# CSU-KangHu/HiTE

Measured on AMD Instinct MI355X. Metric: candidate TE boundaries/sec on 1 Gbp synthetic genome (fine stage: copy finding+gather+align+vote+judge), higher is better.
Workload: dtype u8; 1 GPU; C3: 1000 Mbp synthetic genome, 2500 TIR + 2500 LTR families, 50000 candidates/GPU judged as TIR (copy finding by minimizer-index lookup inside the timed step; index build 0.0 s untimed); genome_bp=1000000000, candidates_per_gpu=50000, candidate_bases=192511237, copies=799813, copy_table=found, is_te=34225, parallelism=replicated genome, candidates per rank x1, all-gather of 32-B calls

## Files before the change

hite_amd/_lib.py:

```python
import ctypes as C
import os

import numpy as np

_HERE = os.path.dirname(os.path.abspath(__file__))
SO_PATH = os.path.join(_HERE, "libhite_gpu.so")

HITE_TE = {"tir": 0, "helitron": 1, "non_ltr": 2}
INFO = {0: "", 1: "nb", 2: "fl1", 3: "EXC"}
HITE_SUBCLUSTER_CHUNK = 64


class HiteError(RuntimeError):
    pass


class HiteCall(C.Structure):
    _fields_ = [("is_te", C.c_int32), ("info", C.c_int32), ("row_num", C.c_int32), ("bstart", C.c_int32),
                ("bend", C.c_int32), ("cons_len", C.c_int32), ("cons_off", C.c_int64)]


CALL_DTYPE = np.dtype([("is_te", "<i4"), ("info", "<i4"), ("row_num", "<i4"), ("bstart", "<i4"), ("bend", "<i4"),
                       ("cons_len", "<i4"), ("cons_off", "<i8")])
assert CALL_DTYPE.itemsize == 32 and C.sizeof(HiteCall) == 32
# ... 151 lines not shown
        return [counts[coff[i]:coff[i + 1]] for i in range(len(msas))]

    def boundary_search(self, msas, pos, side, thr, variant=3, int_thr=None, out_thr=None, win_in=20, win_out=10):
        buf, off, rows, cols = self.pack_msas(msas)
        n = len(msas)
        pos = _arr(pos, np.int32)
        side = _arr([0 if s in (0, "start") else 1 for s in side], np.int32)
        thr = _arr(thr, np.float64)
        it = _arr(int_thr, np.float64) if int_thr is not None else None
        ot = _arr(out_thr, np.float64) if out_thr is not None else None
        b = np.zeros(n, dtype=np.int32)
        v = np.zeros(n, dtype=np.int32)
        self._check(self.lib.hite_boundary_search(self.h, n, _p(buf), _p(off), _p(rows), _p(cols), _p(pos), _p(side), _p(thr),
                                                  _p(it), _p(ot), int(variant), win_in, win_out, _p(b), _p(v)),
                    "hite_boundary_search")
        return b, v

    def judge(self, te_type, msas, cands, plant=1):
        buf, off, rows, cols = self.pack_msas(msas)
        n = len(msas)
        cb = [c.encode() if isinstance(c, str) else bytes(c) for c in cands]
        coff = np.zeros(n + 1, dtype=np.int64)
        np.cumsum([len(c) for c in cb], out=coff[1:])
        cbuf = np.frombuffer(b"".join(cb) + b"\0" * 16, dtype=np.uint8)
        calls = np.zeros(n, dtype=CALL_DTYPE)
        cons = np.zeros(int(cols.astype(np.int64).sum()) + 8 * n + 16, dtype=np.uint8)
        self._check(self.lib.hite_judge(self.h, HITE_TE[te_type], int(plant), n, _p(buf), _p(off), _p(rows), _p(cols),
                                        _p(cbuf), _p(coff), _p(calls), _p(cons)), "hite_judge")
        out = []
        for i in range(n):
            c = calls[i]
            s = cons[c["cons_off"]:c["cons_off"] + c["cons_len"]].tobytes().decode() if c["is_te"] else ""
            out.append((bool(c["is_te"]), INFO[int(c["info"])], s, int(c["row_num"]), int(c["bstart"]), int(c["bend"])))
        return out

    def tsd_search(self, rows_, bstart, bend, plant=1):
        rb = [r.encode() if isinstance(r, str) else bytes(r) for r in rows_]
        n = len(rb)
        off = np.zeros(n + 1, dtype=np.int64)
        np.cumsum([len(r) for r in rb], out=off[1:])
        buf = np.frombuffer(b"".join(rb) + b"\0" * 16, dtype=np.uint8)
        ln = np.zeros(n, dtype=np.int32)
        lo = np.zeros((n, 16), dtype=np.uint8)
        ro = np.zeros((n, 16), dtype=np.uint8)
        self._check(self.lib.hite_tsd_search(self.h, n, _p(buf), _p(off), _p(_arr(bstart, np.int32)), _p(_arr(bend, np.int32)),
                                             int(plant), _p(ln), _p(lo), _p(ro)), "hite_tsd_search")
        return [(lo[i, :max(ln[i], 0)].tobytes().decode(), ro[i, :max(ln[i], 0)].tobytes().decode(), int(ln[i])) for i in range(n)]

    def align_config(self, exact_cap):
        self._check(self.lib.hite_align_config(self.h, int(exact_cap)), "hite_align_config")

    def align_lanes(self, min_cols):
        self._check(self.lib.hite_align_lanes(self.h, int(min_cols)), "hite_align_lanes")

    def align_stats(self, reset=False):
        o = np.zeros(8, dtype=np.int64)
        self._check(self.lib.hite_align_stats(self.h, _p(o), 1 if reset else 0), "hite_align_stats")
        return dict(zip(("pairs", "certified", "wide", "fallback", "dropped", "cost", "columns", "exact_cap"), (int(x) for x in o)))

    def star_msa(self, groups, sparse=False, info=False):
        flat = [w.encode() if isinstance(w, str) else bytes(w) for g in groups for w in g]
        n = len(groups)
        row_first = np.zeros(n + 1, dtype=np.int32)
        np.cumsum([len(g) for g in groups], out=row_first[1:])
        off = np.zeros(len(flat) + 1, dtype=np.int64)
        np.cumsum([len(w) for w in flat], out=off[1:])
        buf = np.frombuffer(b"".join(flat) + b"\0" * 16, dtype=np.uint8)
        cols = np.zeros(n, dtype=np.int32)
        rows = np.zeros(n, dtype=np.int32)
        inf = np.zeros((len(flat), 5), dtype=np.int32)
        moff = np.zeros(max(n, 1), dtype=np.int64)
        if n == 0:
            return ([], []) if info else []
        ptr = C.POINTER(C.c_uint8)()
        nbytes = C.c_int64(0)
        self._check(self.lib.hite_star_msa_once(self.h, n, _p(buf), _p(off), _p(row_first), 1 if sparse else 0, _p(cols), _p(rows),
                                                _p(inf) if info else None, C.byref(ptr), _p(moff), C.byref(nbytes)), "hite_star_msa_once")
        try:
            out = np.ctypeslib.as_array(ptr, shape=(max(int(nbytes.value), 1),)).copy() if nbytes.value > 0 else np.zeros(1, dtype=np.uint8)
        finally:
            self.lib.hite_host_free(C.cast(ptr, C.c_void_p))
        res = []
        for i in range(n):
            if cols[i] <= 0:
                res.append(None)
            else:
                res.append(out[moff[i]:moff[i] + int(rows[i]) * cols[i]].reshape(int(rows[i]), int(cols[i])).copy())
        if info:
            return res, [inf[row_first[i]:row_first[i + 1]].copy() for i in range(n)]
        return res

    def flank_region_align(self, te_type, cands, copies, plant=1, flank=50):
        n = len(cands)
        cb = [c.encode() if isinstance(c, str) else bytes(c) for c in cands]
        coff = np.zeros(n + 1, dtype=np.int64)
        np.cumsum([len(c) for c in cb], out=coff[1:])
        cbuf = np.frombuffer(b"".join(cb) + b"\0" * 16, dtype=np.uint8)
        cf = np.zeros(n + 1, dtype=np.int32)
        np.cumsum([len(c) for c in copies], out=cf[1:])
        flat = [t for c in copies for t in c]
        contig = _arr([t[0] for t in flat], np.int32)
        s1 = _arr([t[1] for t in flat], np.int64)
        e1 = _arr([t[2] for t in flat], np.int64)
        mn = _arr([t[3] for t in flat], np.uint8)
        has = [len(t) > 5 for t in flat]
        if any(has) and not all(has):
# ... 619 lines not shown
```

hite_amd/csrc/hite_align.hip:

```cpp
#include "hite_common.h"
#include "hite_scan.h"
#include "hite_arena.h"
#include "hite_sort.h"
#include "hite_align.h"

#define AL_GAP 3
#define AL_STEER 24
#define AL_MARGIN 48
#define AL_PADR 1056
#define AL_WIDE_NW 64
#define AL_STRIP 16
#define AL_RECB 4096
#define AL_DEFAULT_CAP 8
#define AL_KBINS 2048
#define AL_LANES_MIN_STRIPS 32

struct AlignArgs {
    const uint8_t *win;
    const int64_t *win_off;
    const int32_t *win_len;
    const int32_t *row_first;
    int n_cand;
    const int32_t *row_cand;
    const uint4 *planes;
// ... 1247 lines not shown
        __syncthreads();
    }
    if (fail) { if (lane == 0) P.st[g] = 1; }
    else out.run(i - 1, i, 0x8000u);
}

__global__ void align_flag_kernel(int64_t nrows, const int32_t *__restrict__ order, const int32_t *__restrict__ strips, AlignArgs P,
                                  int what, int level, int cap, int32_t *__restrict__ flag, int32_t *__restrict__ cols) {
    const int64_t x = (int64_t)blockIdx.x * blockDim.x + threadIdx.x;
    if (x >= nrows) return;
    const int g = order[x];
    int f = 0;
    if (strips[g] > 0) {
        if (what == 0) {
            const int u4 = P.U4[g];
            if (P.st[g] == 0 && u4 >= 0 && u4 + AL_GAP * AL_MARGIN <= 32 * AL_GAP * cap) {
                int first = 8;
                while (32 * AL_GAP * first < u4 + AL_GAP * AL_MARGIN) first *= 2;
                const bool cert = P.U[g] <= P.kst[g];
                f = level >= first && !cert;
            }
        } else if (what == 1) f = P.st[g] == 1;
        else {
            const int u4 = P.U4[g];
            const bool esc = P.st[g] == 0 && u4 >= 0 && u4 + AL_GAP * AL_MARGIN <= 32 * AL_GAP * cap && !(P.U[g] <= P.kst[g]);
            f = what == 2 ? esc : !esc;
        }
    }
    flag[x] = f;
    if (cols) cols[x] = f ? P.win_len[g] + 1 : 0;
}
__global__ void align_compact_kernel(int64_t nrows, const int32_t *__restrict__ order, const int32_t *__restrict__ flag,
                                     const int64_t *__restrict__ pos, int32_t *__restrict__ out, const int64_t *__restrict__ colpos,
                                     int64_t *__restrict__ full_off, int32_t *__restrict__ st) {
    const int64_t x = (int64_t)blockIdx.x * blockDim.x + threadIdx.x;
    if (x >= nrows) return;
    if (flag[x]) {
        const int g = order[x];
        out[pos[x]] = g;
        if (full_off) { full_off[g] = colpos[x]; st[g] = 0; }
    }
}
__global__ void __launch_bounds__(256) align_blockmax_kernel(int64_t cnt, const int32_t *__restrict__ list, const int32_t *__restrict__ strips,
                                                             int32_t *__restrict__ bk) {
    const int64_t x = (int64_t)blockIdx.x * 256 + threadIdx.x;
    const int k = wave_max_i32(x < cnt ? strips[list[x]] : 0);
    if ((threadIdx.x & 63) == 0 && x < cnt) bk[x >> 6] = k;
}
__global__ void align_assign_kernel(int64_t cnt, const int32_t *__restrict__ list, const int64_t *__restrict__ boff, char *region,
                                    unsigned long long *__restrict__ rec) {
    const int64_t x = (int64_t)blockIdx.x * blockDim.x + threadIdx.x;
    if (x < cnt) rec[list[x]] = (unsigned long long)(uintptr_t)(region + boff[x >> 6] * (int64_t)AL_RECB + (x & 63) * 32);
}
struct LaneCost { float thread_chain, lane_chain, thread_work, lane_work; };
__device__ __forceinline__ double lane_cost_at(int64_t k, int64_t nb, const int32_t *bk, const int64_t *boff, const LaneCost c) {
    const double chain_l = k > 0 ? (double)bk[0] * c.lane_chain : 0.0, chain_t = k < nb ? (double)bk[k] * c.thread_chain : 0.0;
    const double work = (double)boff[k] * c.lane_work + (double)(boff[nb] - boff[k]) * c.thread_work;
    double t = chain_l > chain_t ? chain_l : chain_t;
    return t > work ? t : work;
}
__global__ void align_long_blocks_kernel(int64_t nb, const int32_t *__restrict__ bk, const int64_t *__restrict__ boff, int64_t fixed_strips,
                                         LaneCost cf, LaneCost ct, int64_t *__restrict__ out) {
    if (blockIdx.x || threadIdx.x) return;
    for (int w = 0; w < 2; w++) {
        int64_t lo = 0, hi = nb;
        if (fixed_strips >= 0) {
            while (lo < hi) { const int64_t mid = (lo + hi) >> 1; if ((int64_t)bk[mid] >= fixed_strips) lo = mid + 1; else hi = mid; }
        } else {
            const LaneCost c = w ? ct : cf;
            while (lo < hi) {
                const int64_t mid = (lo + hi) >> 1;
                const double a = (double)bk[0] * c.lane_chain, wk = (double)boff[mid] * c.lane_work + (double)(boff[nb] - boff[mid]) * c.thread_work;
                const double tc = mid < nb ? (double)bk[mid] * c.thread_chain : 0.0;
                if ((a > wk ? a : wk) < tc) lo = mid + 1; else hi = mid;
            }
            if (lo > 0 && lane_cost_at(lo - 1, nb, bk, boff, c) <= lane_cost_at(lo, nb, bk, boff, c)) lo--;
            if (lo > 0 && (bk[0] < AL_LANES_MIN_STRIPS || lane_cost_at(lo, nb, bk, boff, c) > 0.9 * lane_cost_at(0, nb, bk, boff, c))) lo = 0;
        }
        out[w] = lo;
    }
}
__global__ void __launch_bounds__(256) align_stats_kernel(int64_t total_rows, const int32_t *__restrict__ strips, AlignArgs P, int32_t *__restrict__ row_dead,
                                                          int32_t *__restrict__ cand_status, unsigned long long *__restrict__ acc) {
    __shared__ unsigned long long s_acc[4][7];
    unsigned long long v[7] = {0, 0, 0, 0, 0, 0, 0};
    for (int64_t g = (int64_t)blockIdx.x * blockDim.x + threadIdx.x; g < total_rows; g += (int64_t)gridDim.x * blockDim.x) {
        if (strips[g] <= 0) {
            const bool empty_row = g != P.row_first[P.row_cand[g]];
            if (empty_row) { P.st[g] = 2; P.U[g] = -1; P.kst[g] = -1; P.lvl[g] = 0; v[0] += 1ull; v[4] += 1ull; }
            if (row_dead) row_dead[g] = empty_row;
            if (empty_row && cand_status) atomicExch(&cand_status[P.row_cand[g]], 2);
        }
        else {
            const int st = P.st[g];
            v[0] += 1ull;
            v[1] += st == 0 && P.U[g] <= P.kst[g];
            v[2] += st == 0 && (P.lvl[g] & 0xff) > 4;
            v[3] += (P.lvl[g] & 0x100) != 0;
            v[4] += st != 0;
            v[5] += st == 0 ? (unsigned long long)P.U[g] : 0ull;
            v[6] += (unsigned long long)P.win_len[g];
            if (row_dead) row_dead[g] = st != 0;
            if (st != 0 && cand_status) atomicExch(&cand_status[P.row_cand[g]], 2);
        }
    }
#pragma unroll
    for (int q = 0; q < 7; q++) {
        unsigned long long x = v[q];
#pragma unroll
        for (int d = 32; d >= 1; d >>= 1) x += __shfl_xor(x, d, 64);
        if ((threadIdx.x & 63) == 0) s_acc[threadIdx.x >> 6][q] = x;
    }
    __syncthreads();
    if (threadIdx.x < 7) {
        const unsigned long long x = s_acc[0][threadIdx.x] + s_acc[1][threadIdx.x] + s_acc[2][threadIdx.x] + s_acc[3][threadIdx.x];
        if (x) atomicAdd(&acc[threadIdx.x], x);
    }
}
__global__ void align_info_kernel(int64_t total_rows, AlignArgs P, int32_t *__restrict__ info ) {
    const int64_t g = (int64_t)blockIdx.x * blockDim.x + threadIdx.x;
    if (g >= total_rows) return;
    const int c = P.row_cand[g];
    if (g == P.row_first[c]) { for (int q = 0; q < 5; q++) info[g * 5 + q] = 0; return; }
    info[g * 5 + 0] = P.U[g];
    info[g * 5 + 1] = P.st[g] != 2 && P.U[g] <= P.kst[g];
    info[g * 5 + 2] = P.st[g];
    info[g * 5 + 3] = P.kst[g];
    info[g * 5 + 4] = P.lvl[g];
}

struct AlignState {
    Arena arena;
    int64_t *h_pin = nullptr;
    int64_t *d_scal = nullptr;
    int exact_cap = -1;
    int lanes_min = -1;
    float lanes_scale[4] = {1.f, 1.f, 1.f, 1.f};
    bool sort_attr = false;
    hipStream_t st2 = nullptr;
    hipEvent_t ev = nullptr, ev_fork = nullptr, ev_join = nullptr;
    int64_t stats[8] = {0, 0, 0, 0, 0, 0, 0, 0};
};

static hipError_t align_make_stream(hipStream_t *out) {
    int lo = 0, hi = 0;
    if (hipDeviceGetStreamPriorityRange(&lo, &hi) != hipSuccess) { lo = 0; hi = 0; }
    return hipStreamCreateWithPriority(out, hipStreamNonBlocking, hi);
}

static AlignState *align_state(hite_ctx *ctx) {
    if (!ctx->align_state) {
        AlignState *S = new AlignState();
        if (hipHostMalloc((void **)&S->h_pin, 64 * sizeof(int64_t)) != hipSuccess || hipMalloc((void **)&S->d_scal, 64 * sizeof(int64_t)) != hipSuccess ||
            align_make_stream(&S->st2) != hipSuccess || hipEventCreateWithFlags(&S->ev, hipEventDisableTiming) != hipSuccess ||
            hipEventCreateWithFlags(&S->ev_fork, hipEventDisableTiming) != hipSuccess || hipEventCreateWithFlags(&S->ev_join, hipEventDisableTiming) != hipSuccess) {
            delete S;
            return nullptr;
        }
        const char *e = getenv("HITE_ALIGN_EXACT");
        int cap = e && *e ? atoi(e) : AL_DEFAULT_CAP;
        if (cap != 0 && cap != 8 && cap != 16 && cap != 32) cap = AL_DEFAULT_CAP;
        S->exact_cap = cap;
        const char *l = getenv("HITE_ALIGN_LANES");
        if (l && *l) { const int v = atoi(l); S->lanes_min = v < -2 ? -1 : v; }
        const char *sc = getenv("HITE_ALIGN_LANES_SCALE");
        if (sc && *sc) sscanf(sc, "%f,%f,%f,%f", &S->lanes_scale[0], &S->lanes_scale[1], &S->lanes_scale[2], &S->lanes_scale[3]);
        ctx->align_state = S;
    }
    return (AlignState *)ctx->align_state;
}
void hite_align_release(hite_ctx *ctx) {
    AlignState *S = (AlignState *)ctx->align_state;
    if (!S) return;
    arena_free(S->arena);
    if (S->h_pin) (void)hipHostFree(S->h_pin);
    if (S->d_scal) (void)hipFree(S->d_scal);
    if (S->st2) (void)hipStreamDestroy(S->st2);
    if (S->ev) (void)hipEventDestroy(S->ev);
    if (S->ev_fork) (void)hipEventDestroy(S->ev_fork);
    if (S->ev_join) (void)hipEventDestroy(S->ev_join);
    delete S;
    ctx->align_state = nullptr;
}

extern "C" int hite_align_config(hite_ctx *ctx, int32_t exact_cap) {
    if (!ctx || (exact_cap != 0 && exact_cap != 8 && exact_cap != 16 && exact_cap != 32)) return HITE_EINVAL;
    AlignState *S = align_state(ctx);
    if (!S) return HITE_ENOMEM;
    S->exact_cap = exact_cap;
    return HITE_OK;
}
extern "C" int hite_align_lanes(hite_ctx *ctx, int32_t min_cols) {
    if (!ctx || min_cols < -2 || min_cols > 32767) return HITE_EINVAL;
    AlignState *S = align_state(ctx);
    if (!S) return HITE_ENOMEM;
    S->lanes_min = min_cols;
    return HITE_OK;
}
extern "C" int hite_align_stats(hite_ctx *ctx, int64_t *out8, int32_t reset) {
    if (!ctx || !out8) return HITE_EINVAL;
    AlignState *S = align_state(ctx);
    if (!S) return HITE_ENOMEM;
    memcpy(out8, S->stats, sizeof S->stats);
    out8[7] = S->exact_cap;
    if (reset) memset(S->stats, 0, sizeof S->stats);
    return HITE_OK;
}

#define ACHK(x) do { int rc__ = (x); if (rc__) return rc__; } while (0)

template <typename T>
static int aalloc(hite_ctx *ctx, Arena &A, size_t count, T **out) {
    void *p = nullptr;
    int rc = arena_alloc(ctx, A, count * sizeof(T), &p);
    *out = (T *)p;
    return rc;
}

static int build_list(hite_ctx *ctx, AlignState *S, hipStream_t st, int64_t nrows, const int32_t *order, const int32_t *strips,
                      AlignArgs &P, int what, int level, int cap, int32_t *flag, int32_t *cols, int64_t *pos, int64_t *colpos,
                      int64_t *scan_tmp, int32_t *list, int64_t *full_off, int64_t *count, int64_t *total_cols, int slot = 0) {
    const unsigned nb = (unsigned)((nrows + 255) / 256);
    hipLaunchKernelGGL(align_flag_kernel, dim3(nb), dim3(256), 0, st, nrows, order, strips, P, what, level, cap, flag, cols);
    ACHK(scan_excl_buf<int32_t>(ctx, scan_tmp, flag, nrows, pos, st));
    if (cols) ACHK(scan_excl_buf<int32_t>(ctx, scan_tmp, cols, nrows, colpos, st));
    hipLaunchKernelGGL(align_compact_kernel, dim3(nb), dim3(256), 0, st, nrows, order, flag, pos, list, cols ? colpos : nullptr,
                       cols ? full_off : nullptr, P.st);
    HITE_CHECK(ctx, hipMemcpyAsync(S->d_scal + slot, pos + nrows, 8, hipMemcpyDeviceToDevice, st));
    if (cols) HITE_CHECK(ctx, hipMemcpyAsync(S->d_scal + slot + 1, colpos + nrows, 8, hipMemcpyDeviceToDevice, st));
    HITE_CHECK(ctx, hipMemcpyAsync(S->h_pin + slot, S->d_scal + slot, 16, hipMemcpyDeviceToHost, st));
    HITE_CHECK(ctx, hipStreamSynchronize(st));
    *count = S->h_pin[slot];
    if (total_cols) *total_cols = cols ? S->h_pin[slot + 1] : 0;
    return HITE_OK;
}

static int assign_records(hite_ctx *ctx, AlignState *S, hipStream_t st, const int32_t *list, int64_t cnt, const int32_t *strips, int32_t *bk,
                          int64_t *boff, int64_t *scan_tmp, unsigned long long *rec, int slot, int words = 4, int64_t *n_long = nullptr, int64_t *n_long_tb = nullptr) {
    if (n_long) *n_long = 0;
    if (n_long_tb) *n_long_tb = 0;
    if (cnt <= 0) return HITE_OK;
    const int64_t nb = (cnt + 63) / 64;
    hipLaunchKernelGGL(align_blockmax_kernel, dim3((unsigned)((cnt + 255) / 256)), dim3(256), 0, st, cnt, list, strips, bk);
    ACHK(scan_excl_buf<int32_t>(ctx, scan_tmp, bk, nb, boff, st));
    HITE_CHECK(ctx, hipMemcpyAsync(S->d_scal + slot, boff + nb, 8, hipMemcpyDeviceToDevice, st));
    const bool lanes = n_long && S->lanes_min != -2;
    if (lanes) {
        LaneCost fwd4 = {5440.f, 3200.f, 4.3f, 12.5f}, fwd8 = {7040.f, 3200.f, 13.75f, 25.f}, tb = {6880.f, 530.f, 4.3f, 21.5f};
        fwd4.lane_work *= S->lanes_scale[0]; fwd8.lane_work *= S->lanes_scale[1]; tb.lane_work *= S->lanes_scale[2];
        fwd4.lane_chain *= S->lanes_scale[3]; fwd8.lane_chain *= S->lanes_scale[3];
        hipLaunchKernelGGL(align_long_blocks_kernel, dim3(1), dim3(1), 0, st, nb, bk, boff,
                           (int64_t)(S->lanes_min < 0 ? -1 : (S->lanes_min + AL_STRIP - 1) / AL_STRIP), words == 4 ? fwd4 : fwd8, tb, S->d_scal + slot + 1);
    }
    HITE_CHECK(ctx, hipMemcpyAsync(S->h_pin + slot, S->d_scal + slot, 24, hipMemcpyDeviceToHost, st));
    HITE_CHECK(ctx, hipStreamSynchronize(st));
    const int64_t block_strips = S->h_pin[slot];
    if (lanes) {
        const int64_t v = S->h_pin[slot + 1] * 64, vt = S->h_pin[slot + 2] * 64;
        *n_long = v < cnt ? v : cnt;
        if (n_long_tb) *n_long_tb = vt < cnt ? vt : cnt;
    }
    char *region;
    ACHK(aalloc(ctx, S->arena, (size_t)block_strips * AL_RECB + 256, &region));
    hipLaunchKernelGGL(align_assign_kernel, dim3((unsigned)((cnt + 255) / 256)), dim3(256), 0, st, cnt, list, boff, region, rec);
    return HITE_OK;
}

int hite_align_run(hite_ctx *ctx, int32_t n_cand, const uint8_t *d_win, const int64_t *d_win_off, const int32_t *d_win_len,
                   const int32_t *d_row_first, int64_t total_rows, const int64_t *d_ops_base, uint16_t *d_ops,
                   int32_t *d_row_dead, int32_t *d_cand_flag, int32_t *d_info, const char *tag, hipStream_t st) {
    if (!ctx || n_cand < 0 || total_rows < 0 || total_rows > 0x7fffffff) return HITE_EINVAL;
    if (n_cand == 0 || total_rows == 0) return HITE_OK;
    AlignState *S = align_state(ctx);
    if (!S) return HITE_ENOMEM;
    Arena &A = S->arena;
    ACHK(arena_reset(ctx, A, true));
    const int cap = S->exact_cap;
    AlignArgs P;
    memset(&P, 0, sizeof P);
    P.win = d_win; P.win_off = d_win_off; P.win_len = d_win_len; P.row_first = d_row_first; P.n_cand = n_cand;
    P.ops_base = d_ops_base; P.ops = d_ops;
    int32_t *row_cand, *strips, *order, *pwords, *flag, *flag2, *cols, *list, *list_esc, *list_fin;
    unsigned long long *skeys;
    int64_t *plane_off, *pos, *pos2, *colpos, *scan_tmp, *scan_tmp2, *full_off, *boff, *boff2;
    int32_t *bk, *bk2;
    unsigned long long *rec;
    ACHK(aalloc(ctx, A, (size_t)total_rows, &row_cand));
    ACHK(aalloc(ctx, A, (size_t)total_rows, &strips));
    ACHK(aalloc(ctx, A, (size_t)total_rows + 1, &skeys));
    ACHK(aalloc(ctx, A, (size_t)total_rows + 1, &order));
    Sorter srt;
    srt.ctx = ctx; srt.st = st; srt.cap = total_rows; srt.hist_n = sorter_hist_elems(total_rows);
    ACHK(aalloc(ctx, A, (size_t)total_rows + 1, &srt.k2));
    ACHK(aalloc(ctx, A, (size_t)total_rows + 1, &srt.v2));
    ACHK(aalloc(ctx, A, (size_t)srt.hist_n, &srt.hist));
    ACHK(aalloc(ctx, A, (size_t)srt.hist_n + 1, &srt.offs));
    ACHK(aalloc(ctx, A, (size_t)sorter_tmp_elems(srt.hist_n), &srt.bs));
    ACHK(aalloc(ctx, A, (size_t)n_cand, &pwords));
    ACHK(aalloc(ctx, A, (size_t)n_cand + 1, &plane_off));
    ACHK(aalloc(ctx, A, (size_t)total_rows, &rec));
    ACHK(aalloc(ctx, A, (size_t)total_rows / 64 + 2, &bk));
    ACHK(aalloc(ctx, A, (size_t)total_rows / 64 + 3, &boff));
    ACHK(aalloc(ctx, A, (size_t)total_rows / 64 + 2, &bk2));
    ACHK(aalloc(ctx, A, (size_t)total_rows / 64 + 3, &boff2));
    ACHK(aalloc(ctx, A, (size_t)total_rows, &flag));
    ACHK(aalloc(ctx, A, (size_t)total_rows, &cols));
    ACHK(aalloc(ctx, A, (size_t)total_rows, &list));
    ACHK(aalloc(ctx, A, (size_t)total_rows, &list_esc));
    ACHK(aalloc(ctx, A, (size_t)total_rows, &list_fin));
    ACHK(aalloc(ctx, A, (size_t)total_rows, &flag2));
    ACHK(aalloc(ctx, A, (size_t)total_rows + 1, &pos2));
    ACHK(aalloc(ctx, A, (size_t)scan_tmp_elems(total_rows) + 16, &scan_tmp2));
    ACHK(aalloc(ctx, A, (size_t)total_rows + 1, &pos));
// ... 10 lines not shown
    HITE_CHECK(ctx, hipMemsetAsync(P.st, 0, (size_t)total_rows * 4, st));
    HITE_CHECK(ctx, hipMemsetAsync(P.lvl, 0, (size_t)total_rows * 4, st));
    hipLaunchKernelGGL(align_rows_kernel, dim3(n_cand), dim3(256), 0, st, n_cand, d_row_first, d_win_len, row_cand, strips, skeys, (unsigned *)order);
    if (!S->sort_attr) {
        HITE_CHECK(ctx, hipFuncSetAttribute(reinterpret_cast<const void *>(rs_scatter_staged_kernel<true>), hipFuncAttributeMaxDynamicSharedMemorySize, RSS_LDS_BYTES));
        S->sort_attr = true;
    }
    ACHK(sorter_sort(srt, skeys, (unsigned *)order, total_rows, 11));
    hipLaunchKernelGGL(align_plane_words_kernel, dim3((n_cand + 255) / 256), dim3(256), 0, st, n_cand, d_row_first, d_win_len, pwords);
    ACHK(scan_excl_buf<int32_t>(ctx, scan_tmp, pwords, n_cand, plane_off, st));
    HITE_CHECK(ctx, hipMemcpyAsync(S->d_scal, plane_off + n_cand, 8, hipMemcpyDeviceToDevice, st));
    HITE_CHECK(ctx, hipMemcpyAsync(S->h_pin, S->d_scal, 8, hipMemcpyDeviceToHost, st));
    int64_t nl4 = 0, nltb = 0;
    ACHK(assign_records(ctx, S, st, order, total_rows, strips, bk, boff, scan_tmp, rec, 1, 4, &nl4, &nltb));
    const int64_t plane_words = S->h_pin[0];
    uint4 *planes;
    ACHK(aalloc(ctx, A, (size_t)plane_words + 8, &planes));
    P.planes = planes; P.plane_off = plane_off; P.rec = rec;
    hipLaunchKernelGGL(align_planes_kernel, dim3(n_cand), dim3(256), 0, st, n_cand, d_win, d_win_off, d_win_len, d_row_first, plane_off, planes);
    hite_prof_end(ctx, tk, st);
    HITE_CHECK(ctx, hipGetLastError());
    char name[32];
    const int nrows = (int)total_rows;
    snprintf(name, sizeof name, "align_fwd4%s", tag ? tag : "");
    hipStream_t s2 = S->st2;
    char lname[40];
    if (getenv("HITE_ALIGN_DEBUG")) fprintf(stderr, "[align%s] rows %d  block-strips %lld  lane-parallel prefix %lld forward, %lld traceback\n", tag ? tag : "", nrows, (long long)S->h_pin[1], (long long)nl4, (long long)nltb);
    if (nl4 > 0) {
        HITE_CHECK(ctx, hipEventRecord(S->ev_fork, st));
        HITE_CHECK(ctx, hipStreamWaitEvent(s2, S->ev_fork, 0));
        snprintf(lname, sizeof lname, "align_fwd4_lanes%s", tag ? tag : "");
        const int tl = hite_prof_begin(ctx, lname, s2);
        hipLaunchKernelGGL(HIP_KERNEL_NAME(align_fwd_lanes_kernel<4>), dim3((unsigned)((nl4 + 15) / 16)), dim3(64), 0, s2, P, order, (int)nl4);
        hite_prof_end(ctx, tl, s2);
        HITE_CHECK(ctx, hipEventRecord(S->ev_join, s2));
    }
    if (nrows > nl4) {
        tk = hite_prof_begin(ctx, name, st);
        hipLaunchKernelGGL(align_fwd4_kernel, dim3((unsigned)((nrows - nl4 + 63) / 64)), dim3(64), 0, st, P, order + nl4, (int)(nrows - nl4));
        hite_prof_end(ctx, tk, st);
    }
    if (nl4 > 0) HITE_CHECK(ctx, hipStreamWaitEvent(st, S->ev_join, 0));
    snprintf(name, sizeof name, "align_tb%s", tag ? tag : "");
    char wname[32];
    snprintf(wname, sizeof wname, "align_fwd_wide%s", tag ? tag : "");
    int64_t n_esc = 0, n_fin = 0;
    const bool overlap = cap >= 16;
    if (cap >= 8 && !overlap) {
        tk = hite_prof_begin(ctx, wname, st);
        for (int level = 8; level <= cap; level *= 2) {
            int64_t cnt = 0;
            ACHK(build_list(ctx, S, st, total_rows, order, strips, P, 0, level, cap, flag, nullptr, pos, colpos, scan_tmp, list, nullptr, &cnt, nullptr));
            if (cnt == 0) continue;
            int64_t nl8 = 0;
            ACHK(assign_records(ctx, S, st, list, cnt, strips, bk, boff, scan_tmp, rec, 1, 8, &nl8));
            if (getenv("HITE_ALIGN_DEBUG")) fprintf(stderr, "[align%s] level %d: pairs %lld  block-strips %lld  lane-parallel prefix %lld\n", tag ? tag : "", level, (long long)cnt, (long long)S->h_pin[1], (long long)nl8);
            if (nl8 > 0) {
                HITE_CHECK(ctx, hipEventRecord(S->ev_fork, st));
                HITE_CHECK(ctx, hipStreamWaitEvent(s2, S->ev_fork, 0));
                snprintf(lname, sizeof lname, "align_fwd_wide_lanes%s", tag ? tag : "");
                const int tl = hite_prof_begin(ctx, lname, s2);
                hipLaunchKernelGGL(HIP_KERNEL_NAME(align_fwd_lanes_kernel<8>), dim3((unsigned)((nl8 + 7) / 8)), dim3(64), 0, s2, P, list, (int)nl8);
                hite_prof_end(ctx, tl, s2);
                HITE_CHECK(ctx, hipEventRecord(S->ev_join, s2));
            }
            if (cnt > nl8)
                hipLaunchKernelGGL(align_fwd8_pair_kernel, dim3((unsigned)((cnt - nl8 + 31) / 32)), dim3(64), 0, st, P, list + nl8, (int)(cnt - nl8));
            if (nl8 > 0) HITE_CHECK(ctx, hipStreamWaitEvent(st, S->ev_join, 0));
        }
        hite_prof_end(ctx, tk, st);
    }
    if (overlap) {
        ACHK(build_list(ctx, S, st, total_rows, order, strips, P, 2, 0, cap, flag, nullptr, pos, colpos, scan_tmp, list_esc, nullptr, &n_esc, nullptr));
        if (n_esc > 0)
            ACHK(build_list(ctx, S, st, total_rows, order, strips, P, 3, 0, cap, flag, nullptr, pos, colpos, scan_tmp, list_fin, nullptr, &n_fin, nullptr));
    }
    if (n_esc > 0) {
        if (n_fin > 0) {
            tk = hite_prof_begin(ctx, name, st);
            hipLaunchKernelGGL(align_tb_kernel, dim3((unsigned)((n_fin + 63) / 64)), dim3(64), 0, st, P, list_fin, (int)n_fin);
            hite_prof_end(ctx, tk, st);
        }
        tk = hite_prof_begin(ctx, wname, s2);
        for (int level = 8; level <= cap; level *= 2) {
            int64_t cnt = 0;
            ACHK(build_list(ctx, S, s2, total_rows, order, strips, P, 0, level, cap, flag2, nullptr, pos2, colpos, scan_tmp2, list, nullptr, &cnt, nullptr, 8));
            if (cnt == 0) continue;
            ACHK(assign_records(ctx, S, s2, list, cnt, strips, bk2, boff2, scan_tmp2, rec, 10));
            const dim3 grid((unsigned)((cnt + 63) / 64));
            if (level == 8) hipLaunchKernelGGL(HIP_KERNEL_NAME(align_fwd_kernel<8>), grid, dim3(64), 0, s2, P, list, (int)cnt);
            else if (level == 16) hipLaunchKernelGGL(HIP_KERNEL_NAME(align_fwd_kernel<16>), grid, dim3(64), 0, s2, P, list, (int)cnt);
            else hipLaunchKernelGGL(HIP_KERNEL_NAME(align_fwd_kernel<32>), grid, dim3(64), 0, s2, P, list, (int)cnt);
        }
        hite_prof_end(ctx, tk, s2);
        HITE_CHECK(ctx, hipEventRecord(S->ev, s2));
        HITE_CHECK(ctx, hipStreamWaitEvent(st, S->ev, 0));
        tk = hite_prof_begin(ctx, name, st);
        hipLaunchKernelGGL(align_tb_kernel, dim3((unsigned)((n_esc + 63) / 64)), dim3(64), 0, st, P, list_esc, (int)n_esc);
        hite_prof_end(ctx, tk, st);
    } else {
        if (nltb > 0) {
            HITE_CHECK(ctx, hipEventRecord(S->ev_fork, st));
            HITE_CHECK(ctx, hipStreamWaitEvent(s2, S->ev_fork, 0));
            snprintf(lname, sizeof lname, "align_tb_strips%s", tag ? tag : "");
            const int tl = hite_prof_begin(ctx, lname, s2);
            hipLaunchKernelGGL(align_tb_strips_kernel, dim3((unsigned)nltb), dim3(64), 0, s2, P, order, (int)nltb);
            hite_prof_end(ctx, tl, s2);
            HITE_CHECK(ctx, hipEventRecord(S->ev_join, s2));
        }
        if (nrows > nltb) {
            tk = hite_prof_begin(ctx, name, st);
            hipLaunchKernelGGL(align_tb_kernel, dim3((unsigned)((nrows - nltb + 63) / 64)), dim3(64), 0, st, P, order + nltb, (int)(nrows - nltb));
            hite_prof_end(ctx, tk, st);
        }
        if (nltb > 0) HITE_CHECK(ctx, hipStreamWaitEvent(st, S->ev_join, 0));
    }
    HITE_CHECK(ctx, hipGetLastError());
    {
        int64_t cnt = 0, tcols = 0;
        ACHK(build_list(ctx, S, st, total_rows, order, strips, P, 1, 0, cap, flag, cols, pos, colpos, scan_tmp, list, full_off, &cnt, &tcols));
        if (cnt > 0) {
// ... 19 lines not shown
```

include/hite_gpu.h:

```cpp
#ifndef HITE_GPU_H
#define HITE_GPU_H
#include <stdint.h>

#ifdef __cplusplus
extern "C" {
#endif

#define HITE_ROW_PAD 0x2e
#define HITE_IS_ROW_PAD(c) (((c) & 0x20u) != 0)

#define HITE_OK 0
#define HITE_EINVAL (-1)
#define HITE_ENOMEM (-2)
#define HITE_EHIP (-3)
#define HITE_ECAP (-4)
#define HITE_ENODEV (-5)

#define HITE_TE_TIR 0
#define HITE_TE_HELITRON 1
#define HITE_TE_NON_LTR 2

#define HITE_INFO_NONE 0
#define HITE_INFO_NB 1
#define HITE_INFO_FL1 2
// ... 116 lines not shown
                        double min_identity, int32_t min_len, int32_t match, int32_t mismatch, int32_t gap_open, int32_t gap_extend,
                        int32_t *d_out, void *stream);

int hite_translate6(hite_ctx *ctx, int64_t n, const uint8_t *nt, const int64_t *nt_off, int64_t cap, uint8_t *aa_out, int64_t *frame_off);
int hite_protein_lib_build(hite_ctx *ctx, int64_t n_prot, const uint8_t *aa, const int64_t *aa_off, void **state_io);
void hite_protein_lib_release(void *state);
int hite_protein_search(hite_ctx *ctx, void *state, int64_t n_query, const uint8_t *nt, const int64_t *nt_off, double evalue, int64_t cap,
                        int32_t *o_query, int32_t *o_prot, int32_t *o_frame, int32_t *o_qstart, int32_t *o_qend, int32_t *o_sstart,
                        int32_t *o_send, int32_t *o_score, int32_t *o_ident, int32_t *o_cols, int64_t *n_out, int64_t *stats);
int hite_protein_smin(int64_t m, int64_t n, double evalue, int32_t *smin);
int hite_protein_tasks(int64_t n, const int32_t *frame, const int32_t *prot, const int32_t *diag, const int32_t *seg_start,
                       const int32_t *seg_end, int64_t n_frames, const int32_t *frame_len, int64_t cap, int32_t *o_frame, int32_t *o_prot,
                       int32_t *o_c, int32_t *o_lo, int32_t *o_hi, int64_t *n_out);
int hite_protein_hsp_filter(int64_t n, const int32_t *score, const int32_t *f_start, const int32_t *p_start, const int32_t *f_end,
                            const int32_t *p_end, uint8_t *keep);

#define HITE_IDENT_MAX_WIDTH 2048
int hite_pair_identity(hite_ctx *ctx, int64_t n_seq, const uint8_t *seqs, const int64_t *seq_off, int64_t n_pair,
                       const int32_t *a_id, const int64_t *a_start, const int64_t *a_end,
                       const int32_t *b_id, const int64_t *b_start, const int64_t *b_end,
                       const uint8_t *strand, int32_t band, int32_t *cost_out, int32_t *match_out);

int hite_copy_index_build(hite_ctx *ctx, void **state_io, void *stream);
int hite_copy_index_forget(void *state);
int hite_copy_config(int32_t aligned_interval);
int hite_copy_config_ctx(hite_ctx *ctx, int32_t aligned_interval);
void hite_copy_index_release(void *state);
int hite_copy_stats(void *state, int64_t out[4]);
int hite_copy_stats_ext(void *state, int64_t out[8]);

int hite_seed_allvsall_dev(hite_ctx *ctx, void **state_io, int64_t seg_len, int64_t max_anchors, int32_t **d_qseg, int32_t **d_sseg,
                           int64_t **d_qs, int64_t **d_qe, int64_t **d_ss, int64_t **d_se, int64_t *n_out, int64_t *stats_out);
int hite_seed_segments(hite_ctx *ctx, int64_t seg_len, int32_t cap, int32_t *seg_chrom, int64_t *seg_off, int32_t *nseg_out);
int hite_seed_shard(hite_ctx *ctx, int32_t rank, int32_t world);
int hite_seed_allvsall(hite_ctx *ctx, void **state_io, int64_t seg_len, int64_t max_anchors, int64_t cap, int32_t *qseg,
                       int32_t *sseg, int64_t *qs, int64_t *qe, int64_t *ss, int64_t *se, int64_t *n_out, int64_t *stats_out);
int hite_find_copies(hite_ctx *ctx, void **state_io, int32_t n_cand, const uint8_t *cand, const int64_t *cand_off,
                     int64_t cap, int32_t *copy_first, int32_t *contig, int64_t *start1, int64_t *end1, uint8_t *minus,
                     int32_t *anchors, int64_t *n_out);
int hite_find_copies_dev(hite_ctx *ctx, void *state, int32_t n_cand, const uint8_t *d_cand, const int64_t *d_cand_off,
                         int64_t cand_bytes, int32_t **d_copy_first, int64_t *n_copies, int32_t **d_contig,
                         int64_t **d_start1, int64_t **d_end1, uint8_t **d_minus, int32_t **d_anchors, void *stream);
int hite_find_copies_restricted_dev(hite_ctx *ctx, void **state_io, int32_t n_cand, const uint8_t *d_cand, const int64_t *d_cand_off,
                                    int64_t cand_bytes, int32_t **d_copy_first, int64_t *n_copies, int32_t **d_contig,
                                    int64_t **d_start1, int64_t **d_end1, uint8_t **d_minus, int32_t **d_anchors, void *stream);
int hite_find_copies_restricted(hite_ctx *ctx, void **state_io, int32_t n_cand, const uint8_t *cand, const int64_t *cand_off,
                                int64_t cap, int32_t *copy_first, int32_t *contig, int64_t *start1, int64_t *end1, uint8_t *minus,
                                int32_t *anchors, int64_t *n_out);
int hite_copy_clips_dev(void *state, const uint32_t **d_clip, int64_t *n);
int hite_copy_clips(void *state, int64_t cap, uint32_t *clip);

int hite_align_config(hite_ctx *ctx, int32_t exact_cap);
int hite_align_lanes(hite_ctx *ctx, int32_t min_cols);
int hite_align_stats(hite_ctx *ctx, int64_t *out8, int32_t reset);
int hite_star_msa(hite_ctx *ctx, int32_t n, const uint8_t *win, const int64_t *win_off, const int32_t *row_first,
                  int32_t *cols_out, int32_t *rows_out, int64_t msa_cap, uint8_t *msa_out, int64_t *msa_off_out);
int hite_star_msa_sparse(hite_ctx *ctx, int32_t n, const uint8_t *win, const int64_t *win_off, const int32_t *row_first,
                         int32_t *cols_out, int32_t *rows_out, int64_t msa_cap, uint8_t *msa_out, int64_t *msa_off_out);
int hite_star_msa_info(hite_ctx *ctx, int32_t n, const uint8_t *win, const int64_t *win_off, const int32_t *row_first,
                       int32_t *cols_out, int32_t *rows_out, int32_t *info_out, int64_t msa_cap, uint8_t *msa_out,
                       int64_t *msa_off_out);
int hite_star_msa_once(hite_ctx *ctx, int32_t n, const uint8_t *win, const int64_t *win_off, const int32_t *row_first,
                       int32_t sparse, int32_t *cols_out, int32_t *rows_out, int32_t *info_out, uint8_t **msa_out,
                       int64_t *msa_off_out, int64_t *msa_bytes_out);
void hite_host_free(void *p);
int hite_star_msa_dev(hite_ctx *ctx, int32_t n, const uint8_t *d_win, const int64_t *d_win_off,
                      const int32_t *d_win_len, const int32_t *d_row_first, int64_t total_rows, const int64_t *d_ops_base, int64_t ops_elems,
                      int32_t max_win_len, int32_t *d_cols_out, int32_t *d_status, int32_t *d_rows_out, void *stream);
int hite_star_msa_fill_dev(hite_ctx *ctx, int32_t n, const uint8_t *d_win, const int64_t *d_win_off,
                           const int32_t *d_win_len, const int32_t *d_row_first, const int64_t *d_ops_base, const int32_t *d_cols,
                           const int64_t *d_msa_off, uint8_t *d_msa, void *stream);
int hite_star_msa_sparse_dev(hite_ctx *ctx, int32_t n, const uint8_t *d_win, const int64_t *d_win_off,
                             const int32_t *d_win_len, const int32_t *d_row_first, int64_t total_rows,
                             const int64_t *d_ops_base, int64_t ops_elems, int32_t max_win_len, int32_t *d_cols_out,
                             int32_t *d_status, int32_t *d_new_cols, int32_t *d_last_extra, int32_t *d_rows_out, void *stream);
int hite_star_msa_fill_sparse_dev(hite_ctx *ctx, int32_t n, const uint8_t *d_win, const int64_t *d_win_off,
                                  const int32_t *d_win_len, const int32_t *d_row_first, const int64_t *d_ops_base,
                                  const int32_t *d_new_cols, const int32_t *d_last_extra, const int64_t *d_msa_off,
                                  uint8_t *d_msa, void *stream);

int hite_flank_region_align(hite_ctx *ctx, int32_t te_type, int32_t plant, int32_t n_cand, const uint8_t *cand,
                            const int64_t *cand_off, const int32_t *copy_first, int64_t n_copies, const int32_t *contig,
                            const int64_t *start1, const int64_t *end1, const uint8_t *minus, int32_t flank,
                            hite_call *calls, uint8_t *cons, int64_t cons_cap, int64_t *stats_out);
int hite_flank_region_align_dev(hite_ctx *ctx, void **state_io, int32_t te_type, int32_t plant, int32_t n_cand,
                                const uint8_t *d_cand, const int64_t *d_cand_off, const int32_t *d_copy_first,
                                int64_t n_copies, const int32_t *d_contig, const int64_t *d_start1, const int64_t *d_end1,
                                const uint8_t *d_minus, int32_t flank, hite_call *d_calls, uint8_t *d_cons,
                                int64_t cons_cap, int64_t *stats_out, void *stream);
int hite_clip_probe(hite_ctx *ctx, int32_t n_cand, const uint8_t *cand, const int64_t *cand_off, const int32_t *copy_first,
                    int64_t n_copies, const int32_t *contig, const int64_t *start1, const int64_t *end1, const uint8_t *minus,
                    uint32_t *clip_out);
int hite_flank_region_align_clip(hite_ctx *ctx, int32_t te_type, int32_t plant, int32_t n_cand, const uint8_t *cand,
                                 const int64_t *cand_off, const int32_t *copy_first, int64_t n_copies, const int32_t *contig,
                                 const int64_t *start1, const int64_t *end1, const uint8_t *minus, const uint32_t *clip, int32_t flank,
                                 hite_call *calls, uint8_t *cons, int64_t cons_cap, int64_t *stats_out);
int hite_flank_region_align_clip_dev(hite_ctx *ctx, void **state_io, int32_t te_type, int32_t plant, int32_t n_cand,
                                     const uint8_t *d_cand, const int64_t *d_cand_off, const int32_t *d_copy_first,
                                     int64_t n_copies, const int32_t *d_contig, const int64_t *d_start1, const int64_t *d_end1,
                                     const uint8_t *d_minus, const uint32_t *d_clip, int32_t flank, hite_call *d_calls,
                                     uint8_t *d_cons, int64_t cons_cap, int64_t *stats_out, void *stream);
void hite_pipeline_release(void *state);

int hite_profile_enable(hite_ctx *ctx, int on);
int hite_profile_reset(hite_ctx *ctx);
int hite_profile_count(hite_ctx *ctx);
// ... 16 lines not shown
```

Before: 673,700 candidates/s.

## Add three-way lane/pair/thread split for wide 8-word forward alignment

Wide (8-word) forward alignment pairs were previously split only into a lane-parallel prefix and a two-lane pair-kernel remainder. A cost model now chooses a three-way split: the longest pairs go to the lane kernel, a middle range to the two-lane pair kernel, and the short tail to a thread-per-pair align_fwd_kernel<8>. The lane and pair kernels run on the second stream concurrently with the thread kernel. The aim is to balance chain length against total work and to overlap the classes, at the cost of a more complex serial split search in a single-thread kernel and cost constants that may be mistuned.

```diff
diff --git a/hite_amd/_lib.py b/hite_amd/_lib.py
--- a/hite_amd/_lib.py
+++ b/hite_amd/_lib.py
@@ -227,6 +227,9 @@
 
     def align_lanes(self, min_cols):
         self._check(self.lib.hite_align_lanes(self.h, int(min_cols)), "hite_align_lanes")
+
+    def align_pair8(self, min_cols):
+        self._check(self.lib.hite_align_pair8(self.h, int(min_cols)), "hite_align_pair8")
 
     def align_stats(self, reset=False):
         o = np.zeros(8, dtype=np.int64)
diff --git a/hite_amd/csrc/hite_align.hip b/hite_amd/csrc/hite_align.hip
--- a/hite_amd/csrc/hite_align.hip
+++ b/hite_amd/csrc/hite_align.hip
@@ -1323,7 +1323,75 @@
     const int64_t x = (int64_t)blockIdx.x * blockDim.x + threadIdx.x;
     if (x < cnt) rec[list[x]] = (unsigned long long)(uintptr_t)(region + boff[x >> 6] * (int64_t)AL_RECB + (x & 63) * 32);
 }
-struct LaneCost { float thread_chain, lane_chain, thread_work, lane_work; };
+struct LaneCost { float thread_chain, lane_chain, thread_work, lane_work, pair_chain, pair_work; };
+__device__ __forceinline__ int64_t first_block_below(int64_t nb, const int32_t *bk, int64_t strips) {
+    int64_t lo = 0, hi = nb;
+    while (lo < hi) { const int64_t mid = (lo + hi) >> 1; if ((int64_t)bk[mid] >= strips) lo = mid + 1; else hi = mid; }
+    return lo;
+}
+__device__ __forceinline__ double level8_chain_at(int64_t nl, int64_t np, int64_t nb, const int32_t *bk, const LaneCost c) {
+    const double cl = nl > 0 ? (double)bk[0] * c.lane_chain : 0.0, cp = np > nl ? (double)bk[nl] * c.pair_chain : 0.0;
+    const double c2 = np < nb ? cl + cp : (cl > cp ? cl : cp), ct = np < nb ? (double)bk[np] * c.thread_chain : 0.0;
+    return c2 > ct ? c2 : ct;
+}
+__device__ __forceinline__ double level8_work_at(int64_t nl, int64_t np, int64_t nb, const int64_t *boff, const LaneCost c) {
+    return (double)boff[nl] * c.lane_work + (double)(boff[np] - boff[nl]) * c.pair_work + (double)(boff[nb] - boff[np]) * c.thread_work;
+}
+__device__ __forceinline__ double level8_cost_at(int64_t nl, int64_t np, int64_t nb, const int32_t *bk, const int64_t *boff, const LaneCost c) {
+    const double ch = level8_chain_at(nl, np, nb, bk, c), wk = level8_work_at(nl, np, nb, boff, c);
+    return ch > wk ? ch : wk;
+}
+__device__ __forceinline__ void level8_best_np(int64_t nl, int64_t nb, const int32_t *bk, const int64_t *boff, const LaneCost c, int64_t *np_out, double *t_out) {
+    int64_t best = nl;
+    double bt = level8_cost_at(nl, nl, nb, bk, boff, c);
+    if (nl < nb && c.pair_work <= c.thread_work) {
+        const double d = level8_cost_at(nl, nb, nb, bk, boff, c);
+        if (d <= bt) { bt = d; best = nb; }
+    } else if (nl < nb) {
+        int64_t lo = nl + 1, hi = nb;
+        while (lo < hi) {
+            const int64_t mid = (lo + hi) >> 1;
+            if (level8_work_at(nl, mid, nb, boff, c) < level8_chain_at(nl, mid, nb, bk, c)) lo = mid + 1; else hi = mid;
+        }
+        const int64_t x = lo;
+        if (x > nl + 1) {
+            const double d = level8_chain_at(nl, x - 1, nb, bk, c);
+            int64_t l2 = nl + 1, h2 = x - 1;
+            while (l2 < h2) { const int64_t mid = (l2 + h2) >> 1; if (level8_chain_at(nl, mid, nb, bk, c) > d) l2 = mid + 1; else h2 = mid; }
+            const double t = level8_cost_at(nl, l2, nb, bk, boff, c);
+            if (t < bt) { bt = t; best = l2; }
+        }
+        const double t = level8_cost_at(nl, x, nb, bk, boff, c);
+        if (t < bt) { bt = t; best = x; }
+    }
+    *np_out = best; *t_out = bt;
+}
+__device__ __forceinline__ void align_level8_split(int64_t nb, const int32_t *bk, const int64_t *boff, int64_t fix_l, int64_t fix_p, const LaneCost c,
+                                                   int64_t min_lane_strips, int64_t *nl_out, int64_t *np_out) {
+    const int64_t pfix = fix_p >= 0 ? first_block_below(nb, bk, fix_p) : -1;
+    int64_t nl = fix_l >= 0 ? first_block_below(nb, bk, fix_l) : 0;
+    int64_t np = pfix > nl ? pfix : nl;
+    double cur = level8_cost_at(nl, np, nb, bk, boff, c);
+    if (pfix < 0) {
+        int64_t x; double t;
+        level8_best_np(nl, nb, bk, boff, c, &x, &t);
+        if (x > nl && (c.pair_work > c.thread_work ? t <= 0.9 * cur : t <= cur)) { np = x; cur = t; }
+    }
+    if (fix_l < 0 && nb > 0 && bk[0] >= min_lane_strips) {
+        double bt = 0.9 * cur;
+        bool found = false;
+        for (int64_t k = 1; k <= nb; k++) {
+            const double a = (double)bk[0] * c.lane_chain, w = (double)boff[k] * c.lane_work + (double)(boff[nb] - boff[k]) * (c.pair_work < c.thread_work ? c.pair_work : c.thread_work);
+            const double lb = a > w ? a : w;
+            if (found ? lb >= bt : lb > bt) break;
+            int64_t x; double t;
+            if (pfix >= 0) { x = pfix > k ? pfix : k; t = level8_cost_at(k, x, nb, bk, boff, c); }
+            else level8_best_np(k, nb, bk, boff, c, &x, &t);
+            if (found ? t < bt : t <= bt) { bt = t; nl = k; np = x; found = true; }
+        }
+    }
+    *nl_out = nl; *np_out = np;
+}
 __device__ __forceinline__ double lane_cost_at(int64_t k, int64_t nb, const int32_t *bk, const int64_t *boff, const LaneCost c) {
     const double chain_l = k > 0 ? (double)bk[0] * c.lane_chain : 0.0, chain_t = k < nb ? (double)bk[k] * c.thread_chain : 0.0;
     const double work = (double)boff[k] * c.lane_work + (double)(boff[nb] - boff[k]) * c.thread_work;
@@ -1331,8 +1399,14 @@
     return t > work ? t : work;
 }
 __global__ void align_long_blocks_kernel(int64_t nb, const int32_t *__restrict__ bk, const int64_t *__restrict__ boff, int64_t fixed_strips,
-                                         LaneCost cf, LaneCost ct, int64_t *__restrict__ out) {
+                                         int64_t fixed_pair, LaneCost cf, LaneCost ct, int64_t *__restrict__ out) {
     if (blockIdx.x || threadIdx.x) return;
+    if (fixed_pair >= -1) {
+        int64_t nl, np;
+        align_level8_split(nb, bk, boff, fixed_strips, fixed_pair, cf, AL_LANES_MIN_STRIPS, &nl, &np);
+        out[0] = nl; out[1] = 0; out[2] = np;
+        return;
+    }
     for (int w = 0; w < 2; w++) {
         int64_t lo = 0, hi = nb;
         if (fixed_strips >= 0) {
@@ -1406,6 +1480,7 @@
     int64_t *d_scal = nullptr;
     int exact_cap = -1;
     int lanes_min = -1;
+    int pair8_min = -1;
     float lanes_scale[4] = {1.f, 1.f, 1.f, 1.f};
     bool sort_attr = false;
     hipStream_t st2 = nullptr;
@@ -1434,6 +1509,8 @@
         S->exact_cap = cap;
         const char *l = getenv("HITE_ALIGN_LANES");
         if (l && *l) { const int v = atoi(l); S->lanes_min = v < -2 ? -1 : v; }
+        const char *p8 = getenv("HITE_ALIGN_PAIR8");
+        if (p8 && *p8) { const int v = atoi(p8); S->pair8_min = v < -2 || v > 32767 ? -1 : v; }
         const char *sc = getenv("HITE_ALIGN_LANES_SCALE");
         if (sc && *sc) sscanf(sc, "%f,%f,%f,%f", &S->lanes_scale[0], &S->lanes_scale[1], &S->lanes_scale[2], &S->lanes_scale[3]);
         ctx->align_state = S;
@@ -1466,6 +1543,13 @@
     AlignState *S = align_state(ctx);
     if (!S) return HITE_ENOMEM;
     S->lanes_min = min_cols;
+    return HITE_OK;
+}
+extern "C" int hite_align_pair8(hite_ctx *ctx, int32_t min_cols) {
+    if (!ctx || min_cols < -2 || min_cols > 32767) return HITE_EINVAL;
+    AlignState *S = align_state(ctx);
+    if (!S) return HITE_ENOMEM;
+    S->pair8_min = min_cols;
     return HITE_OK;
 }
 extern "C" int hite_align_stats(hite_ctx *ctx, int64_t *out8, int32_t reset) {
@@ -1507,29 +1591,35 @@
 }
 
 static int assign_records(hite_ctx *ctx, AlignState *S, hipStream_t st, const int32_t *list, int64_t cnt, const int32_t *strips, int32_t *bk,
-                          int64_t *boff, int64_t *scan_tmp, unsigned long long *rec, int slot, int words = 4, int64_t *n_long = nullptr, int64_t *n_long_tb = nullptr) {
+                          int64_t *boff, int64_t *scan_tmp, unsigned long long *rec, int slot, int words = 4, int64_t *n_long = nullptr, int64_t *n_long_tb = nullptr,
+                          int64_t *n_pair = nullptr) {
     if (n_long) *n_long = 0;
     if (n_long_tb) *n_long_tb = 0;
+    if (n_pair) *n_pair = 0;
     if (cnt <= 0) return HITE_OK;
     const int64_t nb = (cnt + 63) / 64;
     hipLaunchKernelGGL(align_blockmax_kernel, dim3((unsigned)((cnt + 255) / 256)), dim3(256), 0, st, cnt, list, strips, bk);
     ACHK(scan_excl_buf<int32_t>(ctx, scan_tmp, bk, nb, boff, st));
     HITE_CHECK(ctx, hipMemcpyAsync(S->d_scal + slot, boff + nb, 8, hipMemcpyDeviceToDevice, st));
-    const bool lanes = n_long && S->lanes_min != -2;
+    const bool split8 = n_long && n_pair && words == 8;
+    const bool lanes = n_long && (split8 || S->lanes_min != -2);
     if (lanes) {
-        LaneCost fwd4 = {5440.f, 3200.f, 4.3f, 12.5f}, fwd8 = {7040.f, 3200.f, 13.75f, 25.f}, tb = {6880.f, 530.f, 4.3f, 21.5f};
+        LaneCost fwd4 = {5440.f, 3200.f, 4.3f, 12.5f, 0.f, 0.f}, fwd8 = {8600.f, 3200.f, 14.6f, 25.f, 6700.f, 11.6f}, tb = {6880.f, 530.f, 4.3f, 21.5f, 0.f, 0.f};
         fwd4.lane_work *= S->lanes_scale[0]; fwd8.lane_work *= S->lanes_scale[1]; tb.lane_work *= S->lanes_scale[2];
         fwd4.lane_chain *= S->lanes_scale[3]; fwd8.lane_chain *= S->lanes_scale[3];
-        hipLaunchKernelGGL(align_long_blocks_kernel, dim3(1), dim3(1), 0, st, nb, bk, boff,
-                           (int64_t)(S->lanes_min < 0 ? -1 : (S->lanes_min + AL_STRIP - 1) / AL_STRIP), words == 4 ? fwd4 : fwd8, tb, S->d_scal + slot + 1);
-    }
-    HITE_CHECK(ctx, hipMemcpyAsync(S->h_pin + slot, S->d_scal + slot, 24, hipMemcpyDeviceToHost, st));
+        const int64_t never = (int64_t)1 << 30;
+        const int64_t fix_l = S->lanes_min == -2 ? never : S->lanes_min < 0 ? -1 : (S->lanes_min + AL_STRIP - 1) / AL_STRIP;
+        const int64_t fix_p = !split8 ? -2 : S->pair8_min == -2 ? never : S->pair8_min < 0 ? -1 : (S->pair8_min + AL_STRIP - 1) / AL_STRIP;
+        hipLaunchKernelGGL(align_long_blocks_kernel, dim3(1), dim3(1), 0, st, nb, bk, boff, fix_l, fix_p, words == 4 ? fwd4 : fwd8, tb, S->d_scal + slot + 1);
+    }
+    HITE_CHECK(ctx, hipMemcpyAsync(S->h_pin + slot, S->d_scal + slot, 32, hipMemcpyDeviceToHost, st));
     HITE_CHECK(ctx, hipStreamSynchronize(st));
     const int64_t block_strips = S->h_pin[slot];
     if (lanes) {
-        const int64_t v = S->h_pin[slot + 1] * 64, vt = S->h_pin[slot + 2] * 64;
+        const int64_t v = S->h_pin[slot + 1] * 64, vt = S->h_pin[slot + 2] * 64, vp = S->h_pin[slot + 3] * 64;
         *n_long = v < cnt ? v : cnt;
         if (n_long_tb) *n_long_tb = vt < cnt ? vt : cnt;
+        if (split8) *n_pair = vp < *n_long ? *n_long : vp < cnt ? vp : cnt;
     }
     char *region;
     ACHK(aalloc(ctx, S->arena, (size_t)block_strips * AL_RECB + 256, &region));
@@ -1646,21 +1736,31 @@
             int64_t cnt = 0;
             ACHK(build_list(ctx, S, st, total_rows, order, strips, P, 0, level, cap, flag, nullptr, pos, colpos, scan_tmp, list, nullptr, &cnt, nullptr));
             if (cnt == 0) continue;
-            int64_t nl8 = 0;
-            ACHK(assign_records(ctx, S, st, list, cnt, strips, bk, boff, scan_tmp, rec, 1, 8, &nl8));
-            if (getenv("HITE_ALIGN_DEBUG")) fprintf(stderr, "[align%s] level %d: pairs %lld  block-strips %lld  lane-parallel prefix %lld\n", tag ? tag : "", level, (long long)cnt, (long long)S->h_pin[1], (long long)nl8);
-            if (nl8 > 0) {
+            int64_t nl8 = 0, np8 = 0;
+            ACHK(assign_records(ctx, S, st, list, cnt, strips, bk, boff, scan_tmp, rec, 1, 8, &nl8, nullptr, &np8));
+            if (getenv("HITE_ALIGN_DEBUG")) fprintf(stderr, "[align%s] level %d: pairs %lld  block-strips %lld  lane-parallel prefix %lld  two-lane %lld  thread-per-pair %lld\n", tag ? tag : "", level, (long long)cnt, (long long)S->h_pin[1], (long long)nl8, (long long)(np8 - nl8), (long long)(cnt - np8));
+            const bool pair_beside = np8 > nl8 && cnt > np8;
+            const bool fork = nl8 > 0 || pair_beside;
+            if (fork) {
                 HITE_CHECK(ctx, hipEventRecord(S->ev_fork, st));
                 HITE_CHECK(ctx, hipStreamWaitEvent(s2, S->ev_fork, 0));
+            }
+            if (nl8 > 0) {
                 snprintf(lname, sizeof lname, "align_fwd_wide_lanes%s", tag ? tag : "");
                 const int tl = hite_prof_begin(ctx, lname, s2);
                 hipLaunchKernelGGL(HIP_KERNEL_NAME(align_fwd_lanes_kernel<8>), dim3((unsigned)((nl8 + 7) / 8)), dim3(64), 0, s2, P, list, (int)nl8);
                 hite_prof_end(ctx, tl, s2);
-                HITE_CHECK(ctx, hipEventRecord(S->ev_join, s2));
-            }
-            if (cnt > nl8)
-                hipLaunchKernelGGL(align_fwd8_pair_kernel, dim3((unsigned)((cnt - nl8 + 31) / 32)), dim3(64), 0, st, P, list + nl8, (int)(cnt - nl8));
-            if (nl8 > 0) HITE_CHECK(ctx, hipStreamWaitEvent(st, S->ev_join, 0));
+            }
+            if (np8 > nl8)
+                hipLaunchKernelGGL(align_fwd8_pair_kernel, dim3((unsigned)((np8 - nl8 + 31) / 32)), dim3(64), 0, pair_beside ? s2 : st, P, list + nl8, (int)(np8 - nl8));
+            if (fork) HITE_CHECK(ctx, hipEventRecord(S->ev_join, s2));
+            if (cnt > np8) {
+                snprintf(lname, sizeof lname, "align_fwd_wide_thread%s", tag ? tag : "");
+                const int tt = hite_prof_begin(ctx, lname, st);
+                hipLaunchKernelGGL(HIP_KERNEL_NAME(align_fwd_kernel<8>), dim3((unsigned)((cnt - np8 + 63) / 64)), dim3(64), 0, st, P, list + np8, (int)(cnt - np8));
+                hite_prof_end(ctx, tt, st);
+            }
+            if (fork) HITE_CHECK(ctx, hipStreamWaitEvent(st, S->ev_join, 0));
         }
         hite_prof_end(ctx, tk, st);
     }
diff --git a/include/hite_gpu.h b/include/hite_gpu.h
--- a/include/hite_gpu.h
+++ b/include/hite_gpu.h
@@ -192,6 +192,7 @@
 
 int hite_align_config(hite_ctx *ctx, int32_t exact_cap);
 int hite_align_lanes(hite_ctx *ctx, int32_t min_cols);
+int hite_align_pair8(hite_ctx *ctx, int32_t min_cols);
 int hite_align_stats(hite_ctx *ctx, int64_t *out8, int32_t reset);
 int hite_star_msa(hite_ctx *ctx, int32_t n, const uint8_t *win, const int64_t *win_off, const int32_t *row_first,
                   int32_t *cols_out, int32_t *rows_out, int64_t msa_cap, uint8_t *msa_out, int64_t *msa_off_out);
```

Result: no change. 674,300 candidates/s (median of 4 runs) (+0.1%).
